# MingSun-Tse/Collaborative-Distillation

Measured on AMD Instinct MI355X. Metric: content megapixels/sec, end-to-end 5-level WCT (16x VGG, 4K content, 2K style), higher is better.
Workload: dtype f32 (f16x3 split-MFMA products, fp32 accumulate); 1 GPU; PytorchWCT/WCT.py --mode 16x, 5-level WCT, 3840x2160 content, 2048x2048 style, alpha=1, style-side work included, images resident in HBM; BASELINE configs[1]; content_total=3840x2160, parallelism=content column strips x1

## Files before the change

collaborative-distillation_amd/csrc/conv3x3_sp.hip:

```cpp
#include "wct_common.h"
#include "conv_f16_dev.h"
#include <cstdlib>

namespace {

constexpr int SPH = 16;
constexpr int SP_NPH = FHW * (SPH + 2);
constexpr int SP_NBLK = (SP_NPH + 63) / 64;
constexpr int SP_NPP = SP_NBLK * 64;
constexpr int SP_ACT_DMA = (SP_NPH * 4 + 63) / 64;
__device__ __forceinline__ int sp_slot(int pix, int q) { return pix * 4 + (q ^ ((pix >> 2) & 3)); }

struct SpArgs {
  const char* in;
  char* out;
  const u32x4* wpk;
  const float* bias;
  const float* inv_scale_ptr;
  float inv_scale;
  int H, W, inW, inH;
  int cin, cout, cin_chunks, cout_pad, groups;
  int tiles_x, tiles_y, up_in, relu;
  unsigned* sat;
};

typedef __attribute__((address_space(3))) void* lds_ptr;

#ifdef WCT_SP_TIMING
__device__ unsigned long long g_sp_t[4];
#define SP_STAMP(i) do { if (threadIdx.x == 0) { __builtin_amdgcn_sched_barrier(0); const unsigned long long t_ = __builtin_amdgcn_s_memtime(); \
                         spt[i] += t_ - sptl; sptl = t_; __builtin_amdgcn_sched_barrier(0); } } while (0)
#else
#define SP_STAMP(i)
#endif

template <int CT, bool POOL, bool OUTF32, bool GROUPS>
__global__ __launch_bounds__(512) void conv3x3_sp_kernel(SpArgs a) {
  extern __shared__ __attribute__((aligned(16))) char smem[];
  constexpr int COW = CT * 32;
  constexpr int NWV = 8, CPW = CT;
  constexpr int STAGE16 = 4 * SP_NPP + 36 * COW;
  constexpr int W_DMA = 36 * COW / 64;
  constexpr int W_PER_WAVE = (W_DMA + NWV - 1) / NWV;
  constexpr int SP_ACT_PER_WAVE = (SP_ACT_DMA + NWV - 1) / NWV;
  u32x4* lds = reinterpret_cast<u32x4*>(smem);
  float* biasL = reinterpret_cast<float*>(lds + 2 * STAGE16);
  const int tid = threadIdx.x, lane = tid & 63, wave = __builtin_amdgcn_readfirstlane(tid >> 6);
  const int li = lane & 31, kh = lane >> 5;
  const int rw = wave, c0 = 0;
  const int ntiles = a.tiles_x * a.tiles_y;
  for (int e = tid; e < a.cout_pad; e += NWV * 64) biasL[e] = a.bias[e];
  const float inv = a.inv_scale_ptr ? *a.inv_scale_ptr : a.inv_scale;
  const size_t in_plane = sp16_plane_bytes(a.inH, a.inW);
  unsigned long long satmask = 0ull;
  const float lob = a.relu ? 0.f : -65504.f;

  size_t poff[SP_ACT_PER_WAVE];
  auto tile_offsets = [&](int tile) {
    const int ty0 = (tile / a.tiles_x) * SPH, tx0 = (tile % a.tiles_x) * FTW;
#pragma unroll
    for (int i = 0; i < SP_ACT_PER_WAVE; ++i) {
      int idx = wave + NWV * i;
      idx = idx < SP_ACT_DMA ? idx : SP_ACT_DMA - 1;
      const int slot_pix = idx * 16 + (lane >> 2);
      const int q = (lane & 3) ^ ((slot_pix >> 2) & 3);
      const int pix = slot_pix < SP_NPH ? slot_pix : SP_NPH - 1;
      const int py = pix / FHW, px = pix - py * FHW;
      int gy = reflect_clamp(ty0 - 1 + py, a.H), gx = reflect_clamp(tx0 - 1 + px, a.W);
      if (a.up_in) { gy >>= 1; gx >>= 1; }
      poff[i] = ((size_t)gy * a.inW + gx) * 64 + q * 16;
    }
  };
  auto issue_slice = [&](int i, int ch, int grp, int stage) {
    u32x4* act = lds + stage * STAGE16;
    u32x4* wgt = act + 4 * SP_NPP;
    {
      int idx = wave + NWV * i;
      idx = idx < SP_ACT_DMA ? idx : SP_ACT_DMA - 1;
      __builtin_amdgcn_global_load_lds(a.in + (size_t)ch * in_plane + poff[i], (lds_ptr)(act + idx * 64), 16, 0, 0);
    }
    if (i < W_PER_WAVE) {
      int idx = wave + NWV * i;
      idx = idx < W_DMA ? idx : W_DMA - 1;
      const u32x4* g;
// ... 283 lines not shown
    const int stage2 = stage == 0 ? 2 : stage - 1;
    if (ch == 0) {
#pragma unroll
      for (int p = 0; p < 2; ++p)
#pragma unroll
        for (int r = 0; r < 16; ++r) acc[0][p][r] = 0.f;
    }
    const u32x4* act = lds + stage * ACT16;
    const u32x4* wgt = wgt_all + ch * WCH16;
#pragma unroll
    for (int tap = 0; tap < 9; ++tap) {
      const int dy = tap / 3, dx = tap - dy * 3;
      f16x8 bh[2], bl[2];
#pragma unroll
      for (int p = 0; p < 2; ++p) {
        const int pix = (rw * 2 + p + dy) * FHW + li + dx;
        bh[p] = __builtin_bit_cast(f16x8, act[sp_slot(pix, 2 * kh)]);
        bl[p] = __builtin_bit_cast(f16x8, act[sp_slot(pix, 2 * kh + 1)]);
      }
      const f16x8 ah = __builtin_bit_cast(f16x8, wgt[((tap * 2 + 0) * 2 + kh) * COW + li]);
      const f16x8 al = __builtin_bit_cast(f16x8, wgt[((tap * 2 + 1) * 2 + kh) * COW + li]);
      if (tap * PPT < NPIECE && have_pend) {
#pragma unroll
        for (int k = 0; k < PPT; ++k)
          if (tap * PPT + k < NPIECE) epilogue_piece(pend, tap * PPT + k, pty0, ptx0);
      }
      if (tap >= 9 - SP_ACT_PER_WAVE && have2) issue_act(tap - (9 - SP_ACT_PER_WAVE), c2, stage2);
#pragma unroll
      for (int term = 0; term < 3; ++term)
#pragma unroll
        for (int p = 0; p < 2; ++p)
          acc[0][p] = __builtin_amdgcn_mfma_f32_32x32x16_f16(term == 2 ? al : ah, term == 1 ? bl[p] : bh[p], acc[0][p], 0, 0, 0);
    }
    have_pend = false;
    if (ch + 1 == nch) {
#pragma unroll
      for (int p = 0; p < 2; ++p) pend[0][p] = acc[0][p];
      int trow_, tcol_;
      tile_rc(tbase + v, a.tiles_x, txm, trow_, tcol_);
      pty0 = trow_ * SPH; ptx0 = tcol_ * FTW; have_pend = true;
    }
    if (!have1) break;
    v = v1; ch = c1; v1 = v2; c1 = c2; have1 = have2;
    stage = stage == 2 ? 0 : stage + 1;
  }
  if (have_pend) {
#pragma unroll
    for (int k = 0; k < NPIECE; ++k) epilogue_piece(pend, k, pty0, ptx0);
  }
  if (satmask != 0ull && lane == 0 && a.sat) sat_raise(a.sat);
}

template <bool OUTF32>
__global__ __launch_bounds__(512) void conv3x3_sp_up_kernel(SpArgs a) {
  extern __shared__ __attribute__((aligned(16))) char smem[];
  constexpr int COW = 32, NWV = 8;
  constexpr int WSL = 32 * COW;
  constexpr int STAGE16 = 4 * SP_NPP + WSL;
  constexpr int W_DMA = WSL / 64, W_PER_WAVE = W_DMA / NWV;
  constexpr int SP_ACT_PER_WAVE = (SP_ACT_DMA + NWV - 1) / NWV;
  u32x4* lds = reinterpret_cast<u32x4*>(smem);
  float* biasL = reinterpret_cast<float*>(lds + 2 * STAGE16);
  const int tid = threadIdx.x, lane = tid & 63, wave = __builtin_amdgcn_readfirstlane(tid >> 6);
  const int li = lane & 31, kh = lane >> 5, rw = wave;
  const int ntiles = a.tiles_x * a.tiles_y;
  for (int e = tid; e < a.cout_pad; e += NWV * 64) biasL[e] = a.bias[e];
  const float inv = a.inv_scale;
  const size_t in_plane = sp16_plane_bytes(a.inH, a.inW);
  unsigned long long satmask = 0ull;
  const float lob = a.relu ? 0.f : -65504.f;

  size_t poff[SP_ACT_PER_WAVE];
  auto tile_offsets = [&](int tile) {
    const int ty0 = (tile / a.tiles_x) * SPH, tx0 = (tile % a.tiles_x) * FTW;
#pragma unroll
    for (int i = 0; i < SP_ACT_PER_WAVE; ++i) {
      int idx = wave + NWV * i;
      idx = idx < SP_ACT_DMA ? idx : SP_ACT_DMA - 1;
      const int slot_pix = idx * 16 + (lane >> 2);
      const int q = (lane & 3) ^ ((slot_pix >> 2) & 3);
      const int pix = slot_pix < SP_NPH ? slot_pix : SP_NPH - 1;
      const int py = pix / FHW, px = pix - py * FHW;
      int gy = ty0 - 1 + py, gx = tx0 - 1 + px;
      gy = gy < 0 ? 0 : (gy >= a.inH ? a.inH - 1 : gy);
      gx = gx < 0 ? 0 : (gx >= a.inW ? a.inW - 1 : gx);
      poff[i] = ((size_t)gy * a.inW + gx) * 64 + q * 16;
    }
  };
  auto issue_slice = [&](int i, int ch, int grp, int stage) {
    u32x4* act = lds + stage * STAGE16;
    u32x4* wgt = act + 4 * SP_NPP;
    {
      int idx = wave + NWV * i;
      idx = idx < SP_ACT_DMA ? idx : SP_ACT_DMA - 1;
      __builtin_amdgcn_global_load_lds(a.in + (size_t)ch * in_plane + poff[i], (lds_ptr)(act + idx * 64), 16, 0, 0);
    }
    if (i < W_PER_WAVE) {
      const int idx = wave + NWV * i;
      const u32x4* g = a.wpk + ((size_t)((ch * 2 + (grp & 1)) * 32 + idx * 2 + (lane >> 5)) * a.cout_pad + (grp >> 1) * 32 + (lane & 31));
      __builtin_amdgcn_global_load_lds(g, (lds_ptr)(wgt + idx * 64), 16, 0, 0);
    }
  };

  constexpr int NPIECE = 16, PPT = 4;
  auto epilogue_piece = [&](const f32x16 (&r)[2][2], int k, int ty0, int tx0, int pgrp) {
    const int b = k & 1, q = ((k >> 1) & 1) | (((k >> 2) & 1) << 1), p = k >> 3, pa = pgrp & 1;
    const int co = (pgrp >> 1) * COW + 8 * q + 4 * kh;
    const f32x4 bias = *reinterpret_cast<const f32x4*>(biasL + co);
    f32x4 x = fma4(f32x4{r[b][p][4 * q], r[b][p][4 * q + 1], r[b][p][4 * q + 2], r[b][p][4 * q + 3]}, inv, bias);
    if (OUTF32 && a.relu) {
#pragma unroll
      for (int e = 0; e < 4; ++e) x[e] = fmaxf(x[e], 0.f);
    }
    const int oy = 2 * (ty0 + rw * 2 + p) + pa, ox = 2 * (tx0 + li) + b;
    const bool ok = oy < a.H && ox < a.W && co < a.cout;
    if constexpr (OUTF32) {
      if (ok) *reinterpret_cast<f32x4*>(reinterpret_cast<float*>(a.out) + ((size_t)oy * a.W + ox) * a.cout + co) = x;
    } else {
#pragma unroll
      for (int e = 0; e < 4; ++e) satmask |= __ballot(x[e] > 65504.f);
      if (!a.relu) {
#pragma unroll
        for (int e = 0; e < 4; ++e) satmask |= __ballot(x[e] < -65504.f);
      }
      const u32x4 w = sp16_pair_exchange_lob(x, lob);
      if (ok) *reinterpret_cast<u32x4*>(a.out + sp16_piece(sp16_plane_bytes(a.H, a.W), (size_t)oy * a.W + ox, co >> 3, kh)) = w;
    }
  };

  f32x16 acc[2][2], pend[2][2];
  const int xq = ntiles >> 3, xr = ntiles & 7, xcd = blockIdx.x & 7;
  const int tbase = xcd < xr ? xcd * (xq + 1) : xr * (xq + 1) + (xcd - xr) * xq;
  const int ngroups = a.groups;
  const int nunits = (xq + (xcd < xr ? 1 : 0)) * ngroups, ustep = gridDim.x >> 3;
  int v = blockIdx.x >> 3, ch = 0, stage = 0;
  if (v >= nunits) return;
  int grp = v % ngroups;
  int tile = tbase + v / ngroups;
  int dma_tile = tile;
  int pgrp = 0, pty0 = 0, ptx0 = 0;
  bool have_pend = false;
  const unsigned txm = tile_div_magic(a.tiles_x);
  tile_offsets(tile);
#pragma unroll
  for (int i = 0; i < SP_ACT_PER_WAVE; ++i) issue_slice(i, 0, grp, 0);
  while (true) {
    int nv = v, ngrp = grp, nch = ch + 1;
    if (nch == a.cin_chunks) { nch = 0; nv = v + ustep; ngrp = nv % ngroups; }
    const bool more = nv < nunits;
    asm volatile("s_waitcnt vmcnt(0) lgkmcnt(0)" ::: "memory");
    __builtin_amdgcn_s_barrier();
    asm volatile("" ::: "memory");
    if (more) {
      const int ntile = nv == v ? tile : tbase + nv / ngroups;
      if (ntile != dma_tile) { tile_offsets(ntile); dma_tile = ntile; }
    }
    if (ch == 0) {
#pragma unroll
      for (int b = 0; b < 2; ++b)
#pragma unroll
        for (int p = 0; p < 2; ++p)
#pragma unroll
          for (int r = 0; r < 16; ++r) acc[b][p][r] = 0.f;
    }
    const u32x4* act = lds + stage * STAGE16;
    const u32x4* wgt = act + 4 * SP_NPP;
    const int pa = grp & 1;
#pragma unroll
    for (int it = 0; it < 6; ++it) {
      const int i = it / 3, dx = it - i * 3;
      f16x8 bh[2], bl[2];
#pragma unroll
      for (int p = 0; p < 2; ++p) {
        const int pix = (rw * 2 + p + pa + i) * FHW + li + dx;
        bh[p] = __builtin_bit_cast(f16x8, act[sp_slot(pix, 2 * kh)]);
        bl[p] = __builtin_bit_cast(f16x8, act[sp_slot(pix, 2 * kh + 1)]);
      }
      if (it < SP_ACT_PER_WAVE && more) issue_slice(it, nch, ngrp, stage ^ 1);
      if (it >= 2 && have_pend) {
#pragma unroll
        for (int k = 0; k < PPT; ++k) epilogue_piece(pend, (it - 2) * PPT + k, pty0, ptx0, pgrp);
      }
#pragma unroll
      for (int b = 0; b < 2; ++b) {
        const int j = dx - b;
        if (j < 0 || j > 1) continue;
        const f16x8 ah = __builtin_bit_cast(f16x8, wgt[((((b * 2 + i) * 2 + j) * 2 + 0) * 2 + kh) * COW + li]);
        const f16x8 al = __builtin_bit_cast(f16x8, wgt[((((b * 2 + i) * 2 + j) * 2 + 1) * 2 + kh) * COW + li]);
#pragma unroll
        for (int term = 0; term < 3; ++term)
#pragma unroll
          for (int p = 0; p < 2; ++p)
            acc[b][p] = __builtin_amdgcn_mfma_f32_32x32x16_f16(term == 2 ? al : ah, term == 1 ? bl[p] : bh[p], acc[b][p], 0, 0, 0);
      }
    }
    have_pend = false;
    if (ch + 1 == a.cin_chunks) {
#pragma unroll
      for (int b = 0; b < 2; ++b)
#pragma unroll
        for (int p = 0; p < 2; ++p) pend[b][p] = acc[b][p];
      int trow_, tcol_;
      tile_rc(tile, a.tiles_x, txm, trow_, tcol_);
      pty0 = trow_ * SPH; ptx0 = tcol_ * FTW; pgrp = grp; have_pend = true;
    }
    if (!more) break;
    if (nv != v) { v = nv; tile = tbase + nv / ngroups; }
    grp = ngrp; ch = nch; stage ^= 1;
  }
  if (have_pend) {
#pragma unroll
    for (int k = 0; k < NPIECE; ++k) epilogue_piece(pend, k, pty0, ptx0, pgrp);
  }
  if (satmask != 0ull && lane == 0 && a.sat) sat_raise(a.sat);
}

template <typename K>
hipError_t launch_sp(K k, const SpArgs& a, size_t lds, hipStream_t s, int threads, char form = 't') {
  hipError_t e = hipFuncSetAttribute(reinterpret_cast<const void*>(k), hipFuncAttributeMaxDynamicSharedMemorySize, (int)lds);
  if (e != hipSuccess) return e;
  const int ntiles = a.tiles_x * a.tiles_y, want = 8 * ((ntiles + 7) / 8) * a.groups, cus = (num_cus() & ~7) > 8 ? (num_cus() & ~7) : 8;
  const int grid = want < cus ? want : cus;
  note_launch_form(form, SPH, (long)ntiles * a.groups, grid);
  hipLaunchKernelGGL(k, dim3(grid), dim3(threads), lds, s, a);
  return hipGetLastError();
}

}

bool conv_sp_supported(const ConvDesc& d) {
  static const int mask = [] { const char* e = wct_debug_env("WCT_SP_DMA_MASK"); return e ? atoi(e) : 31; }();
  const bool pool = d.flags & CONV_POOL_OUT;
  const int fam = d.cout_pad >= 128 ? 16 : d.cout_pad == 64 ? (pool ? 8 : 4) : (pool ? 2 : 1);
  if (!(mask & fam)) return false;
  return d.wpk16 && !(d.flags & (CONV_IN_NCHW3 | CONV_OUT_NCHW3)) && (d.cin % 16) == 0 && d.cout_pad >= 32 && (d.cout % 8) == 0 &&
         d.cout_pad <= 512;
}

bool conv_sp_up_form(const ConvDesc& d, int H, int W) {
  static const int up_env = [] { const char* e = wct_debug_env("WCT_SP_UP"); return e ? atoi(e) : 1; }();
  return up_env && (d.flags & CONV_UP_IN) && d.wup16 && !(d.flags & CONV_POOL_OUT) && !d.inv_scale_ptr && !(H & 1) && !(W & 1) &&
         (d.cout_pad % 32) == 0;
}

hipError_t launch_conv3x3_sp(const ConvDesc& d, const void* in, void* out, int H, int W, hipStream_t s) {
  if (H < 2 || W < 2 || !conv_sp_supported(d) || !(d.flags & CONV_IN_SP16)) return hipErrorInvalidValue;
  SpArgs a;
  a.in = reinterpret_cast<const char*>(in); a.out = reinterpret_cast<char*>(out);
  a.wpk = reinterpret_cast<const u32x4*>(d.wpk16); a.bias = d.bias;
  a.inv_scale_ptr = d.inv_scale_ptr; a.inv_scale = d.inv_scale;
  a.H = H; a.W = W;
  a.up_in = (d.flags & CONV_UP_IN) ? 1 : 0;
  a.inW = a.up_in ? W / 2 : W; a.inH = a.up_in ? H / 2 : H;
  a.cin = d.cin; a.cout = d.cout; a.cin_chunks = d.cin_chunks; a.cout_pad = d.cout_pad;
  a.tiles_x = (W + FTW - 1) / FTW; a.tiles_y = (H + SPH - 1) / SPH;
  a.relu = (d.flags & CONV_NO_RELU) ? 0 : 1;
  a.sat = d.sat;
  const bool pool = d.flags & CONV_POOL_OUT, f32 = !(d.flags & CONV_OUT_SP16);
  if (conv_sp_up_form(d, H, W)) {
    a.wpk = reinterpret_cast<const u32x4*>(d.wup16);
    a.inv_scale = d.inv_scale_up;
    a.tiles_x = (a.inW + FTW - 1) / FTW; a.tiles_y = (a.inH + SPH - 1) / SPH;
    a.groups = 2 * (d.cout_pad / 32);
    const size_t ldsu = (size_t)2 * (4 * SP_NPP + 32 * 32) * 16 + (size_t)d.cout_pad * sizeof(float);
    return f32 ? launch_sp(conv3x3_sp_up_kernel<true>, a, ldsu, s, 512, 'u') : launch_sp(conv3x3_sp_up_kernel<false>, a, ldsu, s, 512, 'u');
  }
  const int ct = (d.cout_pad % 64 == 0) ? 2 : 1;
  a.groups = d.cout_pad / (ct * 32);
  static const int sp3_env = [] { const char* e = wct_debug_env("WCT_SP3"); return e ? atoi(e) : 1; }();
  if (sp3_env && d.cout_pad == 32 && d.cin_chunks <= 2) {
    const size_t lds3 = ((size_t)3 * 4 * SP_NPP + (size_t)d.cin_chunks * 36 * 32) * 16 + (size_t)d.cout_pad * sizeof(float);
    if (pool) return f32 ? launch_sp(conv3x3_sp3_kernel<true, true>, a, lds3, s, 512, '3') : launch_sp(conv3x3_sp3_kernel<true, false>, a, lds3, s, 512, '3');
    return f32 ? launch_sp(conv3x3_sp3_kernel<false, true>, a, lds3, s, 512, '3') : launch_sp(conv3x3_sp3_kernel<false, false>, a, lds3, s, 512, '3');
  }
  const size_t lds = (size_t)2 * (4 * SP_NPP + 36 * ct * 32) * 16 + (size_t)d.cout_pad * sizeof(float);
#define WCT_SP_CASE(CTV, GV)                                                                                          \
  if (ct == CTV && (a.groups > 1) == GV) {                                                                            \
    if (pool) return f32 ? launch_sp(conv3x3_sp_kernel<CTV, true, true, GV>, a, lds, s, 512) : launch_sp(conv3x3_sp_kernel<CTV, true, false, GV>, a, lds, s, 512); \
    return f32 ? launch_sp(conv3x3_sp_kernel<CTV, false, true, GV>, a, lds, s, 512) : launch_sp(conv3x3_sp_kernel<CTV, false, false, GV>, a, lds, s, 512);         \
  }
  WCT_SP_CASE(1, false)
  WCT_SP_CASE(2, false)
  WCT_SP_CASE(2, true)
#undef WCT_SP_CASE
  return hipErrorInvalidValue;
}

#ifdef WCT_SP_TIMING
extern "C" int wct_debug_sp_timing(unsigned long long* out4) {
  unsigned long long z[4] = {0, 0, 0, 0};
  if (hipMemcpyFromSymbol(out4, HIP_SYMBOL(g_sp_t), sizeof(z)) != hipSuccess) return -1;
  return hipMemcpyToSymbol(HIP_SYMBOL(g_sp_t), z, sizeof(z)) == hipSuccess ? 0 : -1;
}
#endif
```

collaborative-distillation_amd/csrc/wct_api.hip:

```cpp
#include "../../include/wct_hip.h"
#include "../../include/wct_hip_color.h"
#include "../../include/wct_hip_smooth.h"
#include "../../include/wct_hip_swap.h"
#include "../../include/wct_hip_transform.h"
#include "wct_common.h"

#include <cmath>
#include <cstdarg>
#include <cstdlib>
#include <cstdio>
#include <atomic>
#include <cstring>
#include <dlfcn.h>
#include <map>
#include <mutex>
#include <string>
#include <vector>

namespace {

struct DevBuf {
  void* p = nullptr;
  size_t cap = 0;
};
// ... 1175 lines not shown
    ctx->eig_skip = (int)value; ctx->eig_calls = 0;
  }
  else if (!strcmp(key, "swap_key_chunk")) {
    if (!getenv("WCT_DEBUG")) return fail(ctx, WCT_ERR_INVALID, "debug_set: 'swap_key_chunk' is a test / measurement key; set WCT_DEBUG to allow it");
    if (value < 0 || value > 2147483647.0 || value != (double)(long)value) return fail(ctx, WCT_ERR_INVALID, "debug_set: 'swap_key_chunk' takes a key count >= 1, or 0 for the default");
    ctx->swap_key_chunk = (int)value;
    return WCT_OK;
  }
  else if (!strcmp(key, "shard_emulate")) {
    if (!getenv("WCT_DEBUG")) return fail(ctx, WCT_ERR_INVALID, "debug_set: 'shard_emulate' produces wrong results by design (timing experiment); set WCT_DEBUG to allow it");
    const int v = (int)value, world = v / 100, rank = v % 100;
    if (v == 0) { if (ctx->shard_emulate) { ctx->shard_emulate = false; ctx->comm_ranks = 1; ctx->comm_rank = 0; } return WCT_OK; }
    if (!ctx->coll_set || (ctx->comm_ranks != 1 && !ctx->shard_emulate)) return fail(ctx, WCT_ERR_STATE, "debug_set: 'shard_emulate' needs a ONE-rank communicator on the context");
    if (world < 2 || rank >= world) return fail(ctx, WCT_ERR_INVALID, "debug_set: 'shard_emulate' = 100 * ranks + rank");
    ctx->shard_emulate = true; ctx->comm_ranks = world; ctx->comm_rank = rank;
    return WCT_OK;
  }
  else if (!strcmp(key, "side_priority")) {
    int lo = 0, hi = 0;
    HIPCHK(ctx, hipDeviceGetStreamPriorityRange(&lo, &hi));
    HIPCHK(ctx, hipStreamSynchronize(ctx->side.stream));
    hipStream_t ns = nullptr;
    HIPCHK(ctx, hipStreamCreateWithPriority(&ns, hipStreamNonBlocking, value > 0 ? lo : (value < 0 ? hi : 0)));
    (void)hipStreamDestroy(ctx->side.stream);
    ctx->side.stream = ns;
    return WCT_OK;
  }
  else return fail(ctx, WCT_ERR_INVALID, "debug_set: unknown key '%s' (fuse, sp, l1fuse, u8fuse, upconv, fastfold, interleave, foldgemm, nscoop, in3wide, mom32, eig_skip, side_priority, poison, prof_forms, swap_key_chunk)", key);
  HIPCHK(ctx, hipStreamSynchronize(ctx->side.stream));
  return WCT_OK;
}

int wct_debug_get(wct_ctx* ctx, const char* key, double* value) {
  if (!ctx || !key || !value) return WCT_ERR_INVALID;
  WCT_GUARD(ctx);
  if (!strcmp(key, "nscoop_aborts") || !strcmp(key, "nscoop_solves") || !strcmp(key, "nscoop_off")) {
    if (!strcmp(key, "nscoop_solves")) { *value = (double)ctx->main.coop_solves + (double)ctx->side.coop_solves; return WCT_OK; }
    if (!strcmp(key, "nscoop_off")) { (void)coop_usable(ctx, ctx->main); (void)coop_usable(ctx, ctx->side); *value = (ctx->main.coop_off ? 1 : 0) + (ctx->side.coop_off ? 2 : 0); return WCT_OK; }
    HIPCHK(ctx, hipStreamSynchronize(ctx->side.stream));
    HIPCHK(ctx, hipStreamSynchronize(ctx->main.stream));
    unsigned n[2] = {0u, 0u};
    HIPCHK(ctx, hipMemcpy(n, ctx->sat_dev + 2, sizeof n, hipMemcpyDeviceToHost));
    if (ctx->sat_host) { reinterpret_cast<volatile unsigned*>(ctx->sat_host)[2] = n[0]; reinterpret_cast<volatile unsigned*>(ctx->sat_host)[3] = n[1]; }
    *value = (double)n[0] + (double)n[1];
    return WCT_OK;
  }
  if (!strcmp(key, "ws_allocs")) { *value = (double)ctx->ws_allocs; return WCT_OK; }
  if (!strcmp(key, "ws_bytes")) {
    size_t total = 0;
    ctx->each_buf([&](DevBuf& b, Lane*, bool) { total += b.cap; });
    *value = (double)total;
    return WCT_OK;
  }
  return fail(ctx, WCT_ERR_INVALID, "debug_get: unknown key '%s' (nscoop_aborts, nscoop_solves, nscoop_off, ws_allocs, ws_bytes)", key);
}

int wct_load_module(wct_ctx* ctx, int kind, int level, int n_layers, const wct_layer* layers, const float* c0w,
                    const float* c0b) {
  if (!ctx) return WCT_ERR_INVALID;
  WCT_GUARD(ctx);
  if ((kind != WCT_KIND_ENC && kind != WCT_KIND_DEC) || !valid_level(level) || n_layers < 1 || !layers)
    return fail(ctx, WCT_ERR_INVALID, "load_module: bad kind/level/layers (%d, %d, %d)", kind, level, n_layers);
  for (int i = 0; i < n_layers; ++i) {
    const wct_layer& L = layers[i];
    if (!L.weight || !L.bias || L.cin < 1 || L.cout < 1 || L.cin > 512 || L.cout > 512)
      return fail(ctx, WCT_ERR_INVALID, "load_module: layer %d has bad shape %d->%d or NULL weights", i, L.cin, L.cout);
    if (i > 0 && layers[i - 1].cout != L.cin) return fail(ctx, WCT_ERR_INVALID, "load_module: layer %d cin %d != previous cout %d", i, L.cin, layers[i - 1].cout);
    const bool first = i == 0, last = i == n_layers - 1;
    if (kind == WCT_KIND_ENC && first && L.cin != 3) return fail(ctx, WCT_ERR_INVALID, "encoder must start from 3 channels");
    if (kind == WCT_KIND_DEC && last && L.cout != 3) return fail(ctx, WCT_ERR_INVALID, "decoder must end in 3 channels");
    if (!(kind == WCT_KIND_ENC && first) && (L.cin & 3)) return fail(ctx, WCT_ERR_INVALID, "layer %d: cin %d must be a multiple of 4", i, L.cin);
    if (!(kind == WCT_KIND_DEC && last) && (L.cout & 3)) return fail(ctx, WCT_ERR_INVALID, "layer %d: cout %d must be a multiple of 4", i, L.cout);
    for (size_t e = 0; e < (size_t)L.cout * L.cin * 9; ++e)
      if (!std::isfinite(L.weight[e])) return fail(ctx, WCT_ERR_INVALID, "load_module: layer %d has a non-finite weight", i);
    for (int e = 0; e < L.cout; ++e)
      if (!std::isfinite(L.bias[e])) return fail(ctx, WCT_ERR_INVALID, "load_module: layer %d has a non-finite bias", i);
    if (kind == WCT_KIND_ENC && last && L.pool_after) return fail(ctx, WCT_ERR_INVALID, "encoder cannot end in a pool");
    if (kind == WCT_KIND_ENC && first && L.cout > 64)
      return fail(ctx, WCT_ERR_INVALID, "load_module: the first encoder conv has %d output channels; at most 64 are supported", L.cout);
    if (kind == WCT_KIND_ENC && first && L.pool_after) return fail(ctx, WCT_ERR_INVALID, "load_module: the first encoder conv cannot pool");
    if (kind == WCT_KIND_ENC && L.up_after) return fail(ctx, WCT_ERR_INVALID, "load_module: encoder layer %d cannot upsample", i);
    if (kind == WCT_KIND_DEC && L.pool_after) return fail(ctx, WCT_ERR_INVALID, "load_module: decoder layer %d cannot pool", i);
    if (kind == WCT_KIND_DEC && last && L.up_after) return fail(ctx, WCT_ERR_INVALID, "decoder cannot end in an upsample");
  }
  Module& m = ctx->mod[kind][level];
  free_module(m);
  ctx->fold_ready[level] = false;
  m.layers.resize(n_layers);
  for (int i = 0; i < n_layers; ++i) {
    const wct_layer& L = layers[i];
    LayerDev& ld = m.layers[i];
    const bool in3 = kind == WCT_KIND_ENC && i == 0;
    const bool out3 = kind == WCT_KIND_DEC && i == n_layers - 1;
    ld.pool_after = L.pool_after; ld.up_after = L.up_after;
    ld.d.cin = L.cin; ld.d.cout = L.cout;
    ld.d.sat = ctx->sat_dev;
    ld.d.cin_chunks = in3 ? 1 : (L.cin + 15) / 16;
    ld.d.cout_pad = pad_cout(L.cout);
    ld.d.flags = (in3 ? CONV_IN_NCHW3 : 0) | (out3 ? CONV_OUT_NCHW3 : 0) | (L.pool_after ? CONV_POOL_OUT : 0) |
                 ((kind == WCT_KIND_DEC && i > 0 && layers[i - 1].up_after) ? CONV_UP_IN : 0);
    std::vector<float> wpk, bias;
    pack_weights(L.weight, L.bias, L.cout, L.cin, ld.d.cout_pad, in3, in3 ? c0w : nullptr, in3 ? c0b : nullptr, wpk, bias);
    if (int rc = upload(ctx, &ld.wpk, wpk)) return rc;
    if (int rc = upload(ctx, &ld.bias, bias)) return rc;
    ld.d.wpk = ld.wpk; ld.d.bias = ld.bias;
    if (in3 && ld.d.cout_pad <= 32) {
      std::vector<_Float16> w16;
// ... 1599 lines not shown
```

collaborative-distillation_amd/csrc/wct_common.h:

```cpp
#pragma once
#include <hip/hip_runtime.h>
#include <stdint.h>
#include <stddef.h>

#include <stdlib.h>
#include <stdio.h>
#include <vector>

typedef float f32x4 __attribute__((ext_vector_type(4)));
typedef double f64x4 __attribute__((ext_vector_type(4)));

static inline const char* wct_debug_env(const char* name) {
  const char* g = getenv("WCT_DEBUG");
  if (!g || !g[0] || (g[0] == '0' && !g[1])) return nullptr;
  return getenv(name);
}

struct LaunchForm { char form; int tile_h; bool multi; char text[24]; };
extern __thread LaunchForm wct_launch_form __attribute__((visibility("hidden")));
static inline void note_launch_form(char form, int tile_h, long units, long grid) {
  wct_launch_form.form = form; wct_launch_form.tile_h = tile_h; wct_launch_form.multi = units > grid;
}
static inline void note_moments_form(char family, int mp, int nld, int pw, bool pixsplit, bool f32) {
  snprintf(wct_launch_form.text, sizeof wct_launch_form.text, "%c%d.%d.%d%s%c", family, mp, nld, pw, pixsplit ? "s" : "", f32 ? 'f' : 'd');
// ... 2 lines not shown

__device__ __forceinline__ void sat_raise(unsigned* counter) {
  const unsigned old = atomicAdd(counter, 1u);
  if (old >= 0x80000000u) atomicMax(counter, 0x80000000u);
}

struct L1Single { int term, pos; bool zero; };
__host__ __device__ constexpr L1Single l1_single(int s, int kq, int u) {
  const int q = 4 * s + 2 * u + (kq >> 1), j = kq & 1;
  if (q == 15) return L1Single{0, 0, true};
  const int r = q / 5, m = q - 5 * r;
  return m == 0 ? L1Single{0, 3 * r + j, false}
       : m == 1 ? (j == 0 ? L1Single{0, 3 * r + 2, false} : L1Single{2, 3 * r, false})
       : m == 2 ? L1Single{2, 3 * r + 1 + j, false}
       : m == 3 ? L1Single{1, 3 * r + j, false}
                : L1Single{1, 3 * r + 2, j != 0};
}

enum ConvFlags : int {
  CONV_IN_NCHW3 = 1,
  CONV_UP_IN = 2,
  CONV_POOL_OUT = 4,
  CONV_OUT_NCHW3 = 8,
  CONV_NO_RELU = 16,
  CONV_IN_SP16 = 32,
  CONV_OUT_SP16 = 64,
};

struct ConvDesc {
  int cin, cout;
  int cin_chunks;
  int cout_pad;
  int flags;
  const float* wpk;
  const float* bias;
  const void* wpk16 = nullptr;
  float inv_scale = 1.f;
  const float* inv_scale_ptr = nullptr;
  const void* l1w16 = nullptr;
  const float* l1bias = nullptr;
  float l1inv = 1.f;
  const void* wph16 = nullptr;
  const void* wup16 = nullptr;
  float inv_scale_up = 1.f;
  unsigned* sat = nullptr;
};

hipError_t launch_conv3x3(const ConvDesc& d, const float* in, float* out, int H, int W, hipStream_t s);

hipError_t launch_conv3x3_f16(const ConvDesc& d, const float* in, float* out, int H, int W, hipStream_t s);
size_t conv_f16_weight_bytes(int cin, int cout_pad, int taps);
bool conv_sp_supported(const ConvDesc& d);
hipError_t launch_conv3x3_sp(const ConvDesc& d, const void* in, void* out, int H, int W, hipStream_t s);
bool conv_sp_up_form(const ConvDesc& d, int H, int W);
bool conv_fusable_head(const ConvDesc& d0, const ConvDesc& d1);
bool conv_fusable_tail(const ConvDesc& d0, const ConvDesc& d1);
hipError_t launch_enc_head(const ConvDesc& d0, const ConvDesc& d1, const float* img, float* out, int H, int W, hipStream_t s);
hipError_t launch_dec_tail(const ConvDesc& d0, const ConvDesc& d1, const float* in, float* out, int H, int W, hipStream_t s);
bool l1_capable(const ConvDesc& enc0);
bool l1_fusable(const ConvDesc& enc0);
hipError_t launch_l1_encode(const ConvDesc& enc0, const float* img, float* out, int H, int W, hipStream_t s);
hipError_t launch_l1_decode(const ConvDesc& enc0, const ConvDesc& dec0_folded, const float* img, float* out, int H, int W, hipStream_t s);
bool in3_wide_capable(const ConvDesc& enc0);
hipError_t launch_in3_wide(const ConvDesc& enc0, const float* img, void* out, int H, int W, bool out_sp, bool exact_fp32, hipStream_t s);
size_t l1_moments_workspace_bytes();
hipError_t launch_l1_moments(const ConvDesc& enc0, const float* img, int H, int W, int x0, int x1, double* sum, double* sumsq,
                             void* workspace, size_t workspace_bytes, hipStream_t s, bool f32_products = false);
hipError_t launch_split_pack(const float* wpk32, int cin, int cout_pad, int taps, unsigned* maxbits_dev, void* out,
                             float* inv_scale_out, hipStream_t s, bool have_max = false, int nmax = 1);
size_t conv_phase_weight_bytes(int cin);
hipError_t launch_split_pack_phase(const float* wpk32, int cin, const unsigned* maxbits_dev, void* out, hipStream_t s, int nmax = 1);

hipError_t launch_u8_to_planar(const uint8_t* hwc, long npix, float* planar, hipStream_t s);
hipError_t launch_planar_to_u8(const float* planar, long npix, uint8_t* hwc, int round_mode, hipStream_t s);
hipError_t launch_noise_uniform(unsigned long long seed, unsigned stream_id, int H, int W, float* planar, hipStream_t s);
long color_moments_tiles(long npix);
long color_moments_max_pixels();
size_t color_moments_workspace_bytes(long npix);
hipError_t launch_color_moments(const float* planar, long npix, double* sum, double* sumsq, void* workspace, size_t workspace_bytes, hipStream_t s);
hipError_t launch_color_solve(double n_c, const double* sum_c, const double* sumsq_c, double n_s, const double* sum_s, const double* sumsq_s,
                              double eps, double* A, double* t, hipStream_t s);
hipError_t launch_color_apply(const float* in, long npix, const double* A, const double* t, float* out, hipStream_t s);
hipError_t launch_luma_merge(const float* stylised, int Ho, int Wo, const float* content, int Hc, int Wc, float* out_planar, uint8_t* out_hwc,
                             int round_mode, hipStream_t s);
int smooth_vseg(int r);
int smooth_hseg();
size_t smooth_sums_bytes(long npix);
size_t smooth_ab_bytes(long npix);
hipError_t launch_guided_filter(const float* src, int Ho, int Wo, const float* guide, int Hg, int Wg, int r, double eps, float* out_planar,
                                uint8_t* out_hwc, int round_mode, double* sums, size_t sums_bytes, float* ab, size_t ab_bytes, hipStream_t s);
size_t swap_run_bytes(long nq);
size_t swap_norm_bytes(long nk);
hipError_t launch_patch_match(const float* q, int h, int w, const float* k, int hs, int ws, int C, int key_chunk, int32_t* idx, float* best,
                              void* run, size_t run_bytes, float* rnorm, size_t norm_bytes, unsigned* sat, hipStream_t s);
hipError_t launch_patch_assemble(const int32_t* idx, int h, int w, const float* v, int hs, int ws, int C, const float* base, float alpha, float* out,
                                 hipStream_t s);
hipError_t launch_counter_to_f64(const unsigned* counter, double* dst, hipStream_t s);
enum ResizeFilter : int { RESIZE_BILINEAR = 0, RESIZE_BICUBIC = 1 };
void resize_axis_tables(int in_size, int out_size, int filter, int& ksize, std::vector<int>& bounds, std::vector<int>& kk);
hipError_t launch_resize_u8(const uint8_t* in, int H, int W, int oH, int oW, const int* bounds_h, const int* kk_h, int ksize_h,
                            const int* bounds_v_shifted, const int* kk_v, int ksize_v, int row0, int rows, uint8_t* tmp, uint8_t* out,
                            float* planar, hipStream_t s);

hipError_t launch_copy_block(const float* src, long src_pitch, float* dst, long dst_pitch, long rows, int width, hipStream_t s);
struct CopySegs { const float* src[3]; float* dst[3]; long src_pitch[3], dst_pitch[3]; int width[3]; };
hipError_t launch_copy_blocks(const CopySegs& g, long rows, hipStream_t s);
// ... 66 lines not shown
```

Before: 1061 MP/s.

## Add paired-phase upsample conv kernel sharing activation tiles across both row phases

Adds a new form of the fused upsample+3x3 conv kernel in which each work unit computes both output row phases (pa=0,1) from one staged activation tile. The old form gave each phase its own unit, so activations were loaded twice. A resident-weight variant keeps all weight chunks in LDS when there is a single 32-channel group and at most two input chunks. The host picks the paired form when it needs no more than half the scheduling rounds of the split form. In exchange each wave holds twice as many accumulator registers, and the grid has fewer units, which can reduce parallelism.

```diff
diff --git a/collaborative-distillation_amd/csrc/conv3x3_sp.hip b/collaborative-distillation_amd/csrc/conv3x3_sp.hip
--- a/collaborative-distillation_amd/csrc/conv3x3_sp.hip
+++ b/collaborative-distillation_amd/csrc/conv3x3_sp.hip
@@ -1,5 +1,6 @@
 #include "wct_common.h"
 #include "conv_f16_dev.h"
+#include <atomic>
 #include <cstdlib>
 
 namespace {
@@ -30,6 +31,7 @@
 __device__ unsigned long long g_sp_t[4];
 #define SP_STAMP(i) do { if (threadIdx.x == 0) { __builtin_amdgcn_sched_barrier(0); const unsigned long long t_ = __builtin_amdgcn_s_memtime(); \
                          spt[i] += t_ - sptl; sptl = t_; __builtin_amdgcn_sched_barrier(0); } } while (0)
+__device__ unsigned long long g_sp_tu[12];
 #else
 #define SP_STAMP(i)
 #endif
@@ -419,7 +421,7 @@
 }
 
 template <bool OUTF32>
-__global__ __launch_bounds__(512) void conv3x3_sp_up_kernel(SpArgs a) {
+__device__ __forceinline__ unsigned long long sp_up_split(const SpArgs& a) {
   extern __shared__ __attribute__((aligned(16))) char smem[];
   constexpr int COW = 32, NWV = 8;
   constexpr int WSL = 32 * COW;
@@ -501,7 +503,7 @@
   const int ngroups = a.groups;
   const int nunits = (xq + (xcd < xr ? 1 : 0)) * ngroups, ustep = gridDim.x >> 3;
   int v = blockIdx.x >> 3, ch = 0, stage = 0;
-  if (v >= nunits) return;
+  if (v >= nunits) return 0ull;
   int grp = v % ngroups;
   int tile = tbase + v / ngroups;
   int dma_tile = tile;
@@ -511,6 +513,9 @@
   tile_offsets(tile);
 #pragma unroll
   for (int i = 0; i < SP_ACT_PER_WAVE; ++i) issue_slice(i, 0, grp, 0);
+#ifdef WCT_SP_TIMING
+  unsigned long long spt[4] = {0, 0, 0, 0}, sptl = __builtin_amdgcn_s_memtime();
+#endif
   while (true) {
     int nv = v, ngrp = grp, nch = ch + 1;
     if (nch == a.cin_chunks) { nch = 0; nv = v + ustep; ngrp = nv % ngroups; }
@@ -518,6 +523,7 @@
     asm volatile("s_waitcnt vmcnt(0) lgkmcnt(0)" ::: "memory");
     __builtin_amdgcn_s_barrier();
     asm volatile("" ::: "memory");
+    SP_STAMP(0);
     if (more) {
       const int ntile = nv == v ? tile : tbase + nv / ngroups;
       if (ntile != dma_tile) { tile_offsets(ntile); dma_tile = ntile; }
@@ -561,6 +567,7 @@
             acc[b][p] = __builtin_amdgcn_mfma_f32_32x32x16_f16(term == 2 ? al : ah, term == 1 ? bl[p] : bh[p], acc[b][p], 0, 0, 0);
       }
     }
+    SP_STAMP(1);
     have_pend = false;
     if (ch + 1 == a.cin_chunks) {
 #pragma unroll
@@ -571,27 +578,242 @@
       tile_rc(tile, a.tiles_x, txm, trow_, tcol_);
       pty0 = trow_ * SPH; ptx0 = tcol_ * FTW; pgrp = grp; have_pend = true;
     }
+#ifdef WCT_SP_TIMING
+    spt[3] += 1;
+#endif
     if (!more) break;
     if (nv != v) { v = nv; tile = tbase + nv / ngroups; }
     grp = ngrp; ch = nch; stage ^= 1;
+    SP_STAMP(2);
   }
   if (have_pend) {
 #pragma unroll
     for (int k = 0; k < NPIECE; ++k) epilogue_piece(pend, k, pty0, ptx0, pgrp);
   }
-  if (satmask != 0ull && lane == 0 && a.sat) sat_raise(a.sat);
+#ifdef WCT_SP_TIMING
+  SP_STAMP(2);
+  if (threadIdx.x == 0) for (int i = 0; i < 4; ++i) atomicAdd(&g_sp_tu[(a.cin_chunks <= 2 ? 0 : a.cin_chunks <= 4 ? 1 : 2) * 4 + i], spt[i]);
+#endif
+  return satmask;
+}
+
+template <bool OUTF32, bool RES>
+__device__ __forceinline__ unsigned long long sp_up_pair(const SpArgs& a) {
+  extern __shared__ __attribute__((aligned(16))) char smem[];
+  constexpr int COW = 32, NWV = 8;
+  constexpr int ACT16 = 4 * SP_NPP;
+  constexpr int WSL = 32 * COW;
+  constexpr int STAGE16 = RES ? ACT16 : ACT16 + 2 * WSL;
+  constexpr int W_DMA = 2 * WSL / 64, W_PER_WAVE = W_DMA / NWV;
+  constexpr int SP_ACT_PER_WAVE = (SP_ACT_DMA + NWV - 1) / NWV;
+  static_assert(SP_ACT_PER_WAVE + W_PER_WAVE <= 12, "one DMA wave-instruction per patch offset of a job");
+  u32x4* lds = reinterpret_cast<u32x4*>(smem);
+  u32x4* wgt_all = lds + 2 * STAGE16;
+  float* biasL = reinterpret_cast<float*>(wgt_all + (RES ? a.cin_chunks * 2 * WSL : 0));
+  const int tid = threadIdx.x, lane = tid & 63, wave = __builtin_amdgcn_readfirstlane(tid >> 6);
+  const int li = lane & 31, kh = lane >> 5, rw = wave;
+  const int ntiles = a.tiles_x * a.tiles_y;
+  const int nchunks = a.cin_chunks;
+  for (int e = tid; e < a.cout_pad; e += NWV * 64) biasL[e] = a.bias[e];
+  const float inv = a.inv_scale;
+  const size_t in_plane = sp16_plane_bytes(a.inH, a.inW);
+  unsigned long long satmask = 0ull;
+  const float lob = a.relu ? 0.f : -65504.f;
+
+  size_t poff[SP_ACT_PER_WAVE];
+  auto tile_offsets = [&](int tile) {
+    const int ty0 = (tile / a.tiles_x) * SPH, tx0 = (tile % a.tiles_x) * FTW;
+#pragma unroll
+    for (int i = 0; i < SP_ACT_PER_WAVE; ++i) {
+      int idx = wave + NWV * i;
+      idx = idx < SP_ACT_DMA ? idx : SP_ACT_DMA - 1;
+      const int slot_pix = idx * 16 + (lane >> 2);
+      const int q = (lane & 3) ^ ((slot_pix >> 2) & 3);
+      const int pix = slot_pix < SP_NPH ? slot_pix : SP_NPH - 1;
+      const int py = pix / FHW, px = pix - py * FHW;
+      int gy = ty0 - 1 + py, gx = tx0 - 1 + px;
+      gy = gy < 0 ? 0 : (gy >= a.inH ? a.inH - 1 : gy);
+      gx = gx < 0 ? 0 : (gx >= a.inW ? a.inW - 1 : gx);
+      poff[i] = ((size_t)gy * a.inW + gx) * 64 + q * 16;
+    }
+  };
+  auto issue_slice = [&](int s, int ch, int g32, int stage) {
+    u32x4* act = lds + stage * STAGE16;
+    if (s < SP_ACT_PER_WAVE) {
+      int idx = wave + NWV * s;
+      idx = idx < SP_ACT_DMA ? idx : SP_ACT_DMA - 1;
+      __builtin_amdgcn_global_load_lds(a.in + (size_t)ch * in_plane + poff[s], (lds_ptr)(act + idx * 64), 16, 0, 0);
+    } else if (!RES && s < SP_ACT_PER_WAVE + W_PER_WAVE) {
+      const int idx = wave + NWV * (s - SP_ACT_PER_WAVE);
+      const u32x4* g = a.wpk + ((size_t)(ch * 64 + idx * 2 + (lane >> 5)) * a.cout_pad + g32 * 32 + (lane & 31));
+      __builtin_amdgcn_global_load_lds(g, (lds_ptr)(act + ACT16 + idx * 64), 16, 0, 0);
+    }
+  };
+
+  constexpr int NPIECE = 16, PPT = 4;
+  auto epilogue_piece = [&](const f32x16 (&r)[2][2], int k, int ty0, int tx0, int g32, int pa) {
+    const int b = k & 1, q = ((k >> 1) & 1) | (((k >> 2) & 1) << 1), p = k >> 3;
+    const int co = g32 * COW + 8 * q + 4 * kh;
+    const f32x4 bias = *reinterpret_cast<const f32x4*>(biasL + co);
+    f32x4 x = fma4(f32x4{r[b][p][4 * q], r[b][p][4 * q + 1], r[b][p][4 * q + 2], r[b][p][4 * q + 3]}, inv, bias);
+    if (OUTF32 && a.relu) {
+#pragma unroll
+      for (int e = 0; e < 4; ++e) x[e] = fmaxf(x[e], 0.f);
+    }
+    const int oy = 2 * (ty0 + rw * 2 + p) + pa, ox = 2 * (tx0 + li) + b;
+    const bool ok = oy < a.H && ox < a.W && co < a.cout;
+    if constexpr (OUTF32) {
+      if (ok) *reinterpret_cast<f32x4*>(reinterpret_cast<float*>(a.out) + ((size_t)oy * a.W + ox) * a.cout + co) = x;
+    } else {
+#pragma unroll
+      for (int e = 0; e < 4; ++e) satmask |= __ballot(x[e] > 65504.f);
+      if (!a.relu) {
+#pragma unroll
+        for (int e = 0; e < 4; ++e) satmask |= __ballot(x[e] < -65504.f);
+      }
+      const u32x4 w = sp16_pair_exchange_lob(x, lob);
+      if (ok) *reinterpret_cast<u32x4*>(a.out + sp16_piece(sp16_plane_bytes(a.H, a.W), (size_t)oy * a.W + ox, co >> 3, kh)) = w;
+    }
+  };
+
+  f32x16 acc[2][2][2];
+  const int xq = ntiles >> 3, xr = ntiles & 7, xcd = blockIdx.x & 7;
+  const int tbase = xcd < xr ? xcd * (xq + 1) : xr * (xq + 1) + (xcd - xr) * xq;
+  const int ngroups = a.groups;
+  const int nunits = (xq + (xcd < xr ? 1 : 0)) * ngroups, ustep = gridDim.x >> 3;
+  int v = blockIdx.x >> 3, ch = 0, stage = 0;
+  if (v >= nunits) return 0ull;
+  int grp = v % ngroups;
+  int tile = tbase + v / ngroups;
+  int dma_tile = tile;
+  int pgrp = 0, pty0 = 0, ptx0 = 0;
+  bool have_pend = false;
+  const unsigned txm = tile_div_magic(a.tiles_x);
+  if constexpr (RES) {
+    for (int idx = wave; idx < nchunks * W_DMA; idx += NWV) {
+      const u32x4* g = a.wpk + ((size_t)(idx * 2 + (lane >> 5)) * a.cout_pad + (lane & 31));
+      __builtin_amdgcn_global_load_lds(g, (lds_ptr)(wgt_all + idx * 64), 16, 0, 0);
+    }
+  }
+  tile_offsets(tile);
+#pragma unroll
+  for (int s = 0; s < SP_ACT_PER_WAVE + W_PER_WAVE; ++s) issue_slice(s, 0, grp, 0);
+#ifdef WCT_SP_TIMING
+  unsigned long long spt[4] = {0, 0, 0, 0}, sptl = __builtin_amdgcn_s_memtime();
+#endif
+  while (true) {
+    int nv = v, ngrp = grp, nch = ch + 1;
+    if (nch == nchunks) { nch = 0; nv = v + ustep; ngrp = nv % ngroups; }
+    const bool more = nv < nunits, last = ch + 1 == nchunks;
+    asm volatile("s_waitcnt vmcnt(0) lgkmcnt(0)" ::: "memory");
+    __builtin_amdgcn_s_barrier();
+    asm volatile("" ::: "memory");
+    SP_STAMP(0);
+    if (more) {
+      const int ntile = nv == v ? tile : tbase + nv / ngroups;
+      if (ntile != dma_tile) { tile_offsets(ntile); dma_tile = ntile; }
+    }
+    int cty0 = 0, ctx0 = 0;
+    if (last) {
+      int trow_, tcol_;
+      tile_rc(tile, a.tiles_x, txm, trow_, tcol_);
+      cty0 = trow_ * SPH; ctx0 = tcol_ * FTW;
+    }
+    const u32x4* act = lds + stage * STAGE16;
+    const u32x4* wgt = RES ? wgt_all + ch * 2 * WSL : act + ACT16;
+#pragma unroll
+    for (int pa = 0; pa < 2; ++pa) {
+      if (ch == 0) {
+#pragma unroll
+        for (int b = 0; b < 2; ++b)
+#pragma unroll
+          for (int p = 0; p < 2; ++p)
+#pragma unroll
+            for (int r = 0; r < 16; ++r) acc[pa][b][p][r] = 0.f;
+      }
+#pragma unroll
+      for (int it = 0; it < 6; ++it) {
+        const int i = it / 3, dx = it - i * 3;
+        f16x8 bh[2], bl[2];
+#pragma unroll
+        for (int p = 0; p < 2; ++p) {
+          const int pix = (rw * 2 + p + pa + i) * FHW + li + dx;
+          bh[p] = __builtin_bit_cast(f16x8, act[sp_slot(pix, 2 * kh)]);
+          bl[p] = __builtin_bit_cast(f16x8, act[sp_slot(pix, 2 * kh + 1)]);
+        }
+        if (more) issue_slice(pa * 6 + it, nch, ngrp, stage ^ 1);
+        if (it >= 2) {
+          if (pa == 0) {
+            if (have_pend) {
+#pragma unroll
+              for (int k = 0; k < PPT; ++k) epilogue_piece(acc[1], (it - 2) * PPT + k, pty0, ptx0, pgrp, 1);
+            }
+          } else if (last) {
+#pragma unroll
+            for (int k = 0; k < PPT; ++k) epilogue_piece(acc[0], (it - 2) * PPT + k, cty0, ctx0, grp, 0);
+          }
+        }
+#pragma unroll
+        for (int b = 0; b < 2; ++b) {
+          const int j = dx - b;
+          if (j < 0 || j > 1) continue;
+          const f16x8 ah = __builtin_bit_cast(f16x8, wgt[pa * WSL + ((((b * 2 + i) * 2 + j) * 2 + 0) * 2 + kh) * COW + li]);
+          const f16x8 al = __builtin_bit_cast(f16x8, wgt[pa * WSL + ((((b * 2 + i) * 2 + j) * 2 + 1) * 2 + kh) * COW + li]);
+#pragma unroll
+          for (int term = 0; term < 3; ++term)
+#pragma unroll
+            for (int p = 0; p < 2; ++p)
+              acc[pa][b][p] = __builtin_amdgcn_mfma_f32_32x32x16_f16(term == 2 ? al : ah, term == 1 ? bl[p] : bh[p], acc[pa][b][p], 0, 0, 0);
+        }
+      }
+    }
+    SP_STAMP(1);
+    have_pend = last;
+    if (last) { pty0 = cty0; ptx0 = ctx0; pgrp = grp; }
+#ifdef WCT_SP_TIMING
+    spt[3] += 1;
+#endif
+    if (!more) break;
+    if (nv != v) { v = nv; tile = tbase + nv / ngroups; }
+    grp = ngrp; ch = nch; stage ^= 1;
+    SP_STAMP(2);
+  }
+  if (have_pend) {
+#pragma unroll
+    for (int k = 0; k < NPIECE; ++k) epilogue_piece(acc[1], k, pty0, ptx0, pgrp, 1);
+  }
+#ifdef WCT_SP_TIMING
+  SP_STAMP(2);
+  if (threadIdx.x == 0) for (int i = 0; i < 4; ++i) atomicAdd(&g_sp_tu[(a.cin_chunks <= 2 ? 0 : a.cin_chunks <= 4 ? 1 : 2) * 4 + i], spt[i]);
+#endif
+  return satmask;
+}
+
+int sp_grid(int ntiles, int groups) {
+  const int want = 8 * ((ntiles + 7) / 8) * groups, cus = (num_cus() & ~7) > 8 ? (num_cus() & ~7) : 8;
+  return want < cus ? want : cus;
+}
+
+template <bool OUTF32, int FORM>
+__global__ __launch_bounds__(512) void conv3x3_sp_up_kernel(SpArgs a) {
+  unsigned long long satmask;
+  if constexpr (FORM == 0) satmask = sp_up_split<OUTF32>(a);
+  else satmask = sp_up_pair<OUTF32, FORM == 2>(a);
+  if (satmask != 0ull && (threadIdx.x & 63) == 0 && a.sat) sat_raise(a.sat);
 }
 
 template <typename K>
-hipError_t launch_sp(K k, const SpArgs& a, size_t lds, hipStream_t s, int threads, char form = 't') {
+hipError_t launch_sp(K k, const SpArgs& a, size_t lds, hipStream_t s, int threads, char form = 't', int note_groups = 0) {
   hipError_t e = hipFuncSetAttribute(reinterpret_cast<const void*>(k), hipFuncAttributeMaxDynamicSharedMemorySize, (int)lds);
   if (e != hipSuccess) return e;
-  const int ntiles = a.tiles_x * a.tiles_y, want = 8 * ((ntiles + 7) / 8) * a.groups, cus = (num_cus() & ~7) > 8 ? (num_cus() & ~7) : 8;
-  const int grid = want < cus ? want : cus;
-  note_launch_form(form, SPH, (long)ntiles * a.groups, grid);
+  const int ntiles = a.tiles_x * a.tiles_y, grid = sp_grid(ntiles, a.groups);
+  if (note_groups) note_launch_form(form, SPH, (long)ntiles * note_groups, sp_grid(ntiles, note_groups));
+  else note_launch_form(form, SPH, (long)ntiles * a.groups, grid);
   hipLaunchKernelGGL(k, dim3(grid), dim3(threads), lds, s, a);
   return hipGetLastError();
 }
+
+std::atomic<long> g_up_pair_launches{0};
 
 }
 
@@ -603,6 +825,8 @@
   return d.wpk16 && !(d.flags & (CONV_IN_NCHW3 | CONV_OUT_NCHW3)) && (d.cin % 16) == 0 && d.cout_pad >= 32 && (d.cout % 8) == 0 &&
          d.cout_pad <= 512;
 }
+
+long conv_sp_up_pair_launches() { return g_up_pair_launches.load(std::memory_order_relaxed); }
 
 bool conv_sp_up_form(const ConvDesc& d, int H, int W) {
   static const int up_env = [] { const char* e = wct_debug_env("WCT_SP_UP"); return e ? atoi(e) : 1; }();
@@ -628,9 +852,22 @@
     a.wpk = reinterpret_cast<const u32x4*>(d.wup16);
     a.inv_scale = d.inv_scale_up;
     a.tiles_x = (a.inW + FTW - 1) / FTW; a.tiles_y = (a.inH + SPH - 1) / SPH;
-    a.groups = 2 * (d.cout_pad / 32);
-    const size_t ldsu = (size_t)2 * (4 * SP_NPP + 32 * 32) * 16 + (size_t)d.cout_pad * sizeof(float);
-    return f32 ? launch_sp(conv3x3_sp_up_kernel<true>, a, ldsu, s, 512, 'u') : launch_sp(conv3x3_sp_up_kernel<false>, a, ldsu, s, 512, 'u');
+    static const int pair_env = [] { const char* e = wct_debug_env("WCT_SP_UP_PAIR"); return e ? atoi(e) : 1; }();
+    const int ntiles = a.tiles_x * a.tiles_y, g32 = d.cout_pad / 32, tpx = (ntiles + 7) / 8;
+    const int rounds_pair = (tpx * g32 + sp_grid(ntiles, g32) / 8 - 1) / (sp_grid(ntiles, g32) / 8);
+    const int rounds_split = (tpx * 2 * g32 + sp_grid(ntiles, 2 * g32) / 8 - 1) / (sp_grid(ntiles, 2 * g32) / 8);
+    if (pair_env == 2 || (pair_env == 1 && 2 * rounds_pair <= rounds_split)) {
+      a.groups = g32;
+      g_up_pair_launches.fetch_add(1, std::memory_order_relaxed);
+      const bool res = g32 == 1 && d.cin_chunks <= 2;
+      const size_t lds2 = ((size_t)2 * 4 * SP_NPP + (res ? (size_t)d.cin_chunks * 2 * 32 * 32 : (size_t)2 * 2 * 32 * 32)) * 16 +
+                          (size_t)d.cout_pad * sizeof(float);
+      if (res) return f32 ? launch_sp(conv3x3_sp_up_kernel<true, 2>, a, lds2, s, 512, 'u', 2 * g32) : launch_sp(conv3x3_sp_up_kernel<false, 2>, a, lds2, s, 512, 'u', 2 * g32);
+      return f32 ? launch_sp(conv3x3_sp_up_kernel<true, 1>, a, lds2, s, 512, 'u', 2 * g32) : launch_sp(conv3x3_sp_up_kernel<false, 1>, a, lds2, s, 512, 'u', 2 * g32);
+    }
+    a.groups = 2 * g32;
+    const size_t ldsu =(size_t)2 * (4 * SP_NPP + 32 * 32) * 16 + (size_t)d.cout_pad * sizeof(float);
+    return f32 ? launch_sp(conv3x3_sp_up_kernel<true, 0>, a, ldsu, s, 512, 'u') : launch_sp(conv3x3_sp_up_kernel<false, 0>, a, ldsu, s, 512, 'u');
   }
   const int ct = (d.cout_pad % 64 == 0) ? 2 : 1;
   a.groups = d.cout_pad / (ct * 32);
@@ -659,4 +896,9 @@
   if (hipMemcpyFromSymbol(out4, HIP_SYMBOL(g_sp_t), sizeof(z)) != hipSuccess) return -1;
   return hipMemcpyToSymbol(HIP_SYMBOL(g_sp_t), z, sizeof(z)) == hipSuccess ? 0 : -1;
 }
-#endif
+extern "C" int wct_debug_sp_up_timing(unsigned long long* out12) {
+  unsigned long long z[12] = {};
+  if (hipMemcpyFromSymbol(out12, HIP_SYMBOL(g_sp_tu), sizeof(z)) != hipSuccess) return -1;
+  return hipMemcpyToSymbol(HIP_SYMBOL(g_sp_tu), z, sizeof(z)) == hipSuccess ? 0 : -1;
+}
+#endif
diff --git a/collaborative-distillation_amd/csrc/wct_api.hip b/collaborative-distillation_amd/csrc/wct_api.hip
--- a/collaborative-distillation_amd/csrc/wct_api.hip
+++ b/collaborative-distillation_amd/csrc/wct_api.hip
@@ -1251,7 +1251,8 @@
     *value = (double)total;
     return WCT_OK;
   }
-  return fail(ctx, WCT_ERR_INVALID, "debug_get: unknown key '%s' (nscoop_aborts, nscoop_solves, nscoop_off, ws_allocs, ws_bytes)", key);
+  if (!strcmp(key, "sp_up_pair_launches")) { *value = (double)conv_sp_up_pair_launches(); return WCT_OK; }
+  return fail(ctx, WCT_ERR_INVALID, "debug_get: unknown key '%s' (nscoop_aborts, nscoop_solves, nscoop_off, ws_allocs, ws_bytes, sp_up_pair_launches)", key);
 }
 
 int wct_load_module(wct_ctx* ctx, int kind, int level, int n_layers, const wct_layer* layers, const float* c0w,
diff --git a/collaborative-distillation_amd/csrc/wct_common.h b/collaborative-distillation_amd/csrc/wct_common.h
--- a/collaborative-distillation_amd/csrc/wct_common.h
+++ b/collaborative-distillation_amd/csrc/wct_common.h
@@ -78,6 +78,7 @@
 size_t conv_f16_weight_bytes(int cin, int cout_pad, int taps);
 bool conv_sp_supported(const ConvDesc& d);
 hipError_t launch_conv3x3_sp(const ConvDesc& d, const void* in, void* out, int H, int W, hipStream_t s);
+long conv_sp_up_pair_launches();
 bool conv_sp_up_form(const ConvDesc& d, int H, int W);
 bool conv_fusable_head(const ConvDesc& d0, const ConvDesc& d1);
 bool conv_fusable_tail(const ConvDesc& d0, const ConvDesc& d1);
```

Result: no change. 1053 MP/s (-0.8%).
